# Atten4Vis/LW-DETR

Measured on AMD Instinct MI355X. Metric: images/sec, higher is better.
Workload: dtype fp16; 1 GPU; LW-DETR-small inference forward + PostProcess, 640x640, batch 32/GPU, fp16, random-init weights (synthetic COCO-shaped input); global_batch=32, per_gpu_batch=32, parallelism=dp1, collective=none, launch_chains=2

## Files before the change

### include/lwdetr_hip.h

```cpp
#ifndef LWDETR_HIP_H
#define LWDETR_HIP_H
#include <stdint.h>
#ifdef __cplusplus
extern "C" {
#endif

#define LWDETR_OK 0
#define LWDETR_ERR_BAD_ARG (-1)
#define LWDETR_ERR_UNSUPPORTED (-2)
#define LWDETR_ERR_LAUNCH (-3)

int lwdetr_msda_forward(const void* value, const int64_t* shapes, const int64_t* level_start, const void* loc,
                        const void* attn, void* out, int B, int S, int M, int D, int L, int Q, int P, int dtype,
                        void* hip_stream);

int lwdetr_msda_backward(const void* value, const int64_t* shapes, const int64_t* level_start, const void* loc,
                         const void* attn, const void* grad_out, void* grad_value, void* grad_loc, void* grad_attn,
                         int B, int S, int M, int D, int L, int Q, int P, int dtype, void* hip_stream);

int lwdetr_msda_fused_forward(const void* value, const int64_t* shapes, const int64_t* level_start, const void* oa,
                              long ld_oa, int logit_col, const float* ref_boxes, const float* valid_ratios, void* out,
                              int B, int S, int M, int D, int L, int Q, int P, int dtype, void* hip_stream);

typedef struct {
// ... 27 lines not shown
    const float* ln_stats;
    const float* ln_colsum;
} lwdetr_gemm_seg;

typedef struct {
    const void* A; const void* A2;
    const void* W;
    int M, N, K;
    long lda;
    int a_mode;
    lwdetr_tok_layout a_tok;
    int conv_cin, conv_stride, a_col0, conv_hout, conv_wout;
    int img_h, img_w;
    int nseg;
    lwdetr_gemm_seg seg[3];
    void* splitk_ws;
    int splitk;
} lwdetr_gemm_desc;

int lwdetr_gemm(const lwdetr_gemm_desc* desc, int dtype, void* hip_stream);
int lwdetr_gemm_few(const lwdetr_gemm_desc* desc, int dtype, void* hip_stream);
int lwdetr_row_stats(const void* x, long ldx, long M, int C, float eps, float* stats, int dtype, void* hip_stream);
void lwdetr_gemm_tuning(int big_mode);
int lwdetr_has_experiments(void);
void lwdetr_gemm_pt_tuning(int pt_mode);
long lwdetr_gemm_pt_count(void);
int lwdetr_gemm_path_counts(long* out, int n);
const char* lwdetr_gemm_path_name(int i);

typedef struct {
    const void* Q;
    const void* K;
    const void* VT;
    void* out;
    long ldo;
    int B, heads, hd, Tp;
    int seqs_per_img;
    int seq_tok_stride;
    int keys_per_seq;
    int sub_stride, sub_len;
    int kind;
    int vt_slack;
} lwdetr_attn_desc;

int lwdetr_attention(const lwdetr_attn_desc* desc, int dtype, void* hip_stream);
void lwdetr_attention_tuning(int lds_mode);
// ... 122 lines not shown
typedef struct { int kind; int n; int flags; float eps; void* out; long ldo; } lwdetr_chain_stage;
typedef struct {
    const void* in; long ld_in; int k_in;
    const void* res; long ld_res;
    const void* qpos; long ld_q;
    const void* wstream; const float* vec;
    long M; int D; int nst;
    lwdetr_chain_stage st[6];
} lwdetr_chain_desc;
long lwdetr_row_chain_pieces(const lwdetr_chain_desc* desc);
long lwdetr_row_chain_vec_floats(const lwdetr_chain_desc* desc);
int lwdetr_row_chain(const lwdetr_chain_desc* desc, int dtype, void* hip_stream);

long lwdetr_vit_qkv_stream_bytes(int C);
long lwdetr_vit_qkv_vec_floats(int C);
int lwdetr_vit_qkv(const void* x, long ldx, const void* wstream, const float* vec, long M, int C, float eps, void* q_out,
                   void* k_out, void* vt_out, float qscale, int heads, int hd, int Tp, int dtype, void* hip_stream);

long lwdetr_vit_stem_stream_bytes(int C);
long lwdetr_vit_stem_vec_floats(int C);
int lwdetr_vit_stem(const void* img, int B, int img_h, int img_w, int Hp, int Wp, int Twp, const void* pos, long ldpos, void* x,
                    long ldx, const void* wstream, const float* vec, long M, int C, float eps, void* q_out, void* k_out,
                    void* vt_out, float qscale, int heads, int hd, int dtype, void* hip_stream);

int lwdetr_select_gather(const void* om, const void* enc_cls, long ldc, const float* props, const int64_t* idx,
                         void* om_sel, void* logits_out, float* props_sel, int B, int S, int d, int nq, int ncls,
                         int dtype, void* hip_stream);
int lwdetr_decoder_inputs(const void* enc_delta, const float* props_sel, const float* refpoint, const float* valid_ratios,
                          int L, const void* query_feat, const float* dim_t, void* enc_boxes_out, float* ref_out,
                          void* sine_out, void* xdec_out, int B, int nq, int d, int dtype, void* hip_stream);
int lwdetr_box_reparam(const void* delta, const float* ref, long ref_rows, void* out, long R, int dtype, void* hip_stream);
int lwdetr_finalize_outputs(const void* delta, const float* ref, long ref_rows, void* coord_out, long R, const void* logits_pad,
                            long ldc, int ncls, void* logits_out, long out_layer_rows, int dtype, void* hip_stream);

int lwdetr_rowmax(const void* x, long ld, long rows, int ncols, float* out, int dtype, void* hip_stream);
int lwdetr_topk(const void* x, int B, int N, int K, int64_t* idx_out, float* val_out, int dtype, void* hip_stream);
int lwdetr_postprocess(const void* logits, const void* boxes, const float* target_sizes, int B, int nq, int ncls, int K,
                       float* scores, int64_t* labels, float* out_boxes, int dtype, void* hip_stream);
int lwdetr_postprocess_packed(const void* logits, const void* boxes, const float* target_sizes, int B, int nq, int ncls, int K,
                              float* packed, int dtype, void* hip_stream);

#define LWDETR_CRIT_MAX_LAYERS 8
#define LWDETR_MATCH_MAX_NQ 1024
#define LWDETR_CRIT_QCHUNK 32
typedef struct {
    const void* logits;
// ... 145 lines not shown
```

### lw-detr_amd/_native.py

```python
import ctypes as C
import os

import torch

_HERE = os.path.dirname(os.path.abspath(__file__))
LIB_PATH = os.environ.get("LWDETR_HIP_LIB") or os.path.join(_HERE, "liblwdetr_hip.so")
_lib = None

DT_F32, DT_F16, DT_BF16, DT_F64 = 0, 1, 2, 3
A_PLAIN, A_CONV3x3, A_PATCH16 = 0, 1, 2
ACT_NONE, ACT_RELU, ACT_GELU, ACT_SILU = 0, 1, 2, 3
OUT_LINEAR, OUT_HEADS, OUT_HEADS_T, OUT_TOKMAP, OUT_DECONV2x2 = 0, 1, 2, 3, 4
ERR_BAD_ARG, ERR_UNSUPPORTED, ERR_LAUNCH = -1, -2, -3
ERRORS = {-1: "bad argument", -2: "unsupported configuration", -3: "kernel launch failed"}


class NativeError(RuntimeError):
    pass


class TokLayout(C.Structure):
    _fields_ = [("winmajor", C.c_int), ("Hp", C.c_int), ("Wp", C.c_int), ("Twp", C.c_int)]


# ... 135 lines not shown
        l.lwdetr_attention_tuning_cfg.argtypes = [i]
        l.lwdetr_attention_tuning_cfg.restype = None
        l.lwdetr_layernorm.argtypes = [vp, lg, vp, vp, vp, lg, lg, i, f, lg, lg, lg, i, vp]
        l.lwdetr_layernorm_chain.argtypes = [vp, lg, vp, vp, f, vp, lg, vp, vp, f, vp, lg, lg, i, i, vp]
        l.lwdetr_row_stats.argtypes = [vp, lg, lg, i, f, vp, i, vp]
        l.lwdetr_ffn_splits.argtypes = [lg, i, i, i]
        l.lwdetr_ffn_partial.argtypes = [vp, lg, vp, vp, vp, vp, lg, i, i, i, vp]
        l.lwdetr_ffn_finish.argtypes = [vp, lg, vp, i, vp, vp, vp, f, vp, lg, vp, vp, f, vp, lg, lg, i, i, vp]
        l.lwdetr_mlp_fused.argtypes = [vp, lg, vp, vp, vp, vp, vp, vp, lg, vp, lg, i, f, f, vp, lg, vp, vp, vp,
                                       vp, vp, vp, vp, vp, f, i, i, i, i, vp]
        l.lwdetr_vit_block_few.argtypes = [vp, lg, vp, vp, vp, vp, vp, vp, lg, vp, lg, i, f, f, vp, lg, vp, vp, vp,
                                       vp, vp, vp, vp, vp, f, i, i, i, i, vp]
        l.lwdetr_vit_block.argtypes = [vp, lg, vp, lg, vp, vp, vp, lg, vp, lg, i, f, f, i, vp, vp, vp, f, i, i, i, i, vp]
        l.lwdetr_vit_block_stream_bytes.argtypes = [i, i]
        l.lwdetr_vit_block_stream_bytes.restype = C.c_long
        l.lwdetr_vit_block_vec_floats.argtypes = [i]
        l.lwdetr_vit_block_vec_floats.restype = C.c_long
        l.lwdetr_vit_qkv.argtypes = [vp, lg, vp, vp, lg, i, f, vp, vp, vp, f, i, i, i, i, vp]
        l.lwdetr_vit_stem.argtypes = [vp, i, i, i, i, i, i, vp, lg, vp, lg, vp, vp, lg, i, f, vp, vp, vp, f, i, i, i, vp]
        l.lwdetr_vit_stem_stream_bytes.argtypes = [i]
        l.lwdetr_vit_stem_stream_bytes.restype = C.c_long
        l.lwdetr_vit_stem_vec_floats.argtypes = [i]
        l.lwdetr_vit_stem_vec_floats.restype = C.c_long
        l.lwdetr_vit_qkv_stream_bytes.argtypes = [i]
        l.lwdetr_vit_qkv_stream_bytes.restype = C.c_long
        l.lwdetr_vit_qkv_vec_floats.argtypes = [i]
        l.lwdetr_vit_qkv_vec_floats.restype = C.c_long
        l.lwdetr_enc_chain.argtypes = [vp, lg, i, vp, vp, vp, lg, vp, vp, i, vp, vp, vp, vp, lg, i, i, i, i, lg, i, f, f, i, vp]
        l.lwdetr_enc_chain_vec_floats.argtypes = [i, i]
        l.lwdetr_enc_chain_vec_floats.restype = C.c_long
        l.lwdetr_enc_chain_pieces.argtypes = [i, i, i]
        l.lwdetr_enc_chain_pieces.restype = C.c_long
        l.lwdetr_enc_chain_class_cols.argtypes = [i]
        l.lwdetr_enc_chain_class_cols.restype = C.c_long
        l.lwdetr_enc_chain_vec_floats_cls.argtypes = [i, i, i]
        l.lwdetr_enc_chain_vec_floats_cls.restype = C.c_long
        l.lwdetr_enc_chain_pieces_cls.argtypes = [i, i, i, i]
        l.lwdetr_enc_chain_pieces_cls.restype = C.c_long
        l.lwdetr_enc_chain_check.argtypes = [vp, lg, i, vp, vp, vp, lg, vp, vp, i, vp, vp, vp, vp, lg, i, i, i, i, lg, i, i]
        l.lwdetr_row_chain.argtypes = [C.POINTER(ChainDesc), i, vp]
        l.lwdetr_row_chain_pieces.argtypes = [C.POINTER(ChainDesc)]
        l.lwdetr_row_chain_pieces.restype = C.c_long
        l.lwdetr_row_chain_vec_floats.argtypes = [C.POINTER(ChainDesc)]
        l.lwdetr_row_chain_vec_floats.restype = C.c_long
        l.lwdetr_select_gather.argtypes = [vp, vp, lg, vp, vp, vp, vp, vp, i, i, i, i, i, i, vp]
        l.lwdetr_decoder_inputs.argtypes = [vp, vp, vp, vp, i, vp, vp, vp, vp, vp, vp, i, i, i, i, vp]
# ... 210 lines not shown
```

### lw-detr_amd/csrc/common.h

```cpp
#pragma once
#include <hip/hip_runtime.h>
#include <stdint.h>
#include "lwdetr_hip.h"

enum { DT_F32 = 0, DT_F16 = 1, DT_BF16 = 2 };

typedef _Float16 f16;
typedef __bf16 bf16;
typedef float f32x4 __attribute__((ext_vector_type(4)));
typedef float f32x8 __attribute__((ext_vector_type(8)));
typedef float f32x16 __attribute__((ext_vector_type(16)));
typedef _Float16 f16x4 __attribute__((ext_vector_type(4)));
typedef _Float16 f16x8 __attribute__((ext_vector_type(8)));
typedef __bf16 bf16x4 __attribute__((ext_vector_type(4)));
typedef __bf16 bf16x8 __attribute__((ext_vector_type(8)));
typedef short s16x4 __attribute__((ext_vector_type(4)));

template <typename T> struct Vec;
template <> struct Vec<float> { typedef f32x4 v4; typedef f32x8 v8; };
template <> struct Vec<f16> { typedef f16x4 v4; typedef f16x8 v8; };
template <> struct Vec<bf16> { typedef bf16x4 v4; typedef bf16x8 v8; };

template <typename T> __device__ __forceinline__ float to_f32(T x) { return (float)x; }
template <typename T> __device__ __forceinline__ T from_f32(float x) { return (T)x; }
// ... 92 lines not shown
}
__device__ __forceinline__ long tok_encode(int b, int y, int x, const TokLayout& L) {
    if (!L.winmajor) return ((long)b * L.Hp + y) * L.Wp + x;
    const int h = L.Hp >> 2, w = L.Wp >> 2;
    const int wy = y / h, wx = x / w;
    return (long)b * 16 * L.Twp + (wy * 4 + wx) * L.Twp + (y - wy * h) * w + (x - wx * w);
}

enum {
    KID_MSDA = 0, KID_MSDA_GENERIC, KID_MSDA_FUSED, KID_GEMM, KID_GEMM_CONV, KID_GEMM_PATCH, KID_ATTN_WINDOW,
    KID_ATTN_GLOBAL, KID_ATTN_DECODER, KID_LAYERNORM, KID_ELTWISE, KID_MLP, KID_VITBLOCK, KID_CHAIN, KID_COUNT
};
void lwdetr_prof_begin(int kid, double flops, double bytes, hipStream_t s);
void lwdetr_prof_end(hipStream_t s);
struct ProfScope {
    hipStream_t s;
    ProfScope(int kid, double flops, double bytes, hipStream_t st) : s(st) { lwdetr_prof_begin(kid, flops, bytes, st); }
    ~ProfScope() { lwdetr_prof_end(s); }
};

enum {
    KNOB_ATTN_LDS_CFG = 0, KNOB_ATTN_LDS, KNOB_ATTN_SHORT, KNOB_ATTN_WTILE, KNOB_ATTN_WIN, KNOB_ATTN_QT, KNOB_CHAIN_SPLIT_ROWS, KNOB_GEMM_BIG,
    KNOB_GEMM_BIG_BN, KNOB_GEMM_BIG_2WG, KNOB_CONV_PATCH, KNOB_GEMM_TILE, KNOB_GEMM_DMA, KNOB_GEMM_KB, KNOB_GEMM_NST, KNOB_GEMM_PT,
    KNOB_GEMM_PT_SKEW, KNOB_MLP_SMALL_TT, KNOB_FFN_SPLITS, KNOB_MLP_SMALL, KNOB_VB_GRID, KNOB_VB_GELU16, KNOB_VB_HALF, KNOB_GEMM_FEW_WAVES, KNOB_COUNT
};
long lwdetr_knob(int id, long dflt);
bool lwdetr_knob_is_set(int id);

static inline int lwdetr_check_launch() {
    hipError_t e = hipGetLastError();
    return e == hipSuccess ? LWDETR_OK : LWDETR_ERR_LAUNCH;
}

enum {
    GP_PLAIN_64x64 = 0, GP_PLAIN_128x64, GP_PLAIN_128x128,
    GP_RING_64x64_D2, GP_RING_64x64_D3, GP_RING_64x64_D4, GP_RING_64x64_D3_KB64, GP_RING_64x64_SPLITK, GP_RING_128x64, GP_RING_128x128_D3,
    GP_RING_128x128_D4, GP_CONV_PATCH_128, GP_CONV_PATCH_192,
    GP_BIG_256_KB64, GP_BIG_256_KB32, GP_BIG_192_KB64, GP_BIG_128_KB64, GP_BIG_128_KB32, GP_BIG4_256, GP_BIG4_192, GP_BIG_LN,
    GP_PT, GP_FEW_PLAIN, GP_FEW_CONV_KCH4, GP_FEW_CONV_KCH6, GP_COUNT
};
int lwdetr_gemm_path_done(int path, int rc);
```

### lw-detr_amd/csrc/gemm.hip

```cpp
#include "common.h"
#include <cstdlib>
#include <atomic>
#include <type_traits>

int lwdetr_gemm_pt_try(const lwdetr_gemm_desc& d, int dtype, hipStream_t st, bool& taken);

namespace {

constexpr int BK = 32;

template <typename T> __device__ __forceinline__ float act_apply(float x, int act) {
    if (act == ACT_GELU) return gelu_for<T>(x);
    if (act == ACT_SILU) return x * __builtin_amdgcn_rcpf(1.f + __expf(-x));
    if (act == ACT_RELU) return x > 0.f ? x : 0.f;
    return x;
}

__device__ __forceinline__ bool row_offset(const lwdetr_gemm_seg& sg, long m, long& off) {
    if (sg.mode == LWDETR_OUT_LINEAR) { off = m * sg.ldo; return true; }
    if (sg.mode == LWDETR_OUT_HEADS) {
        const int b = (int)(m / sg.p0), t = (int)(m - (long)b * sg.p0);
        off = ((long)b * sg.p2 * sg.p0 + t) * sg.p1;
        return true;
    }
// ... 1344 lines not shown
    if (state[dev] < 0) { (void)hipGetLastError(); return LWDETR_ERR_UNSUPPORTED; }
    static_assert(NW == 8 || lds <= 80 * 1024, "two workgroups per CU");
    const long nwg = ((d.M + BM - 1) / BM) * ((d.N + BN - 1) / BN);
#ifdef LWDETR_EXPERIMENTS
    if constexpr (LN) hipLaunchKernelGGL((gemm_big_ln_kernel<T>), dim3((unsigned)nwg), dim3(512), lds, st, d);
    else if constexpr (NW == 4) hipLaunchKernelGGL((gemm_big4_kernel<T, BN, KB, NST, AMODE>), dim3((unsigned)nwg), dim3(256), lds, st, d);
    else
#endif
    hipLaunchKernelGGL((gemm_big_kernel<T, BN, KB, NST, AMODE>), dim3((unsigned)nwg), dim3(512), lds, st, d);
    constexpr int path = LN ? GP_BIG_LN
                       : NW == 4 ? (BN == 256 ? GP_BIG4_256 : GP_BIG4_192)
                       : BN == 256 ? (KB == 64 ? GP_BIG_256_KB64 : GP_BIG_256_KB32)
                       : BN == 192 ? GP_BIG_192_KB64 : (KB == 64 ? GP_BIG_128_KB64 : GP_BIG_128_KB32);
    static_assert(NW == 4 || BN != 192 || KB == 64, "one 192-wide 8-wave form");
    return lwdetr_gemm_path_done(path, lwdetr_check_launch());
}

int g_big_mode = -1;
template <int AMODE>
bool big_2wg_pays(const lwdetr_gemm_desc& d, int bn) {
    (void)d; (void)bn;
    return false;
}
template <typename T, int AMODE>
int try_launch_big(const lwdetr_gemm_desc& d, hipStream_t st, bool& taken) {
    taken = false;
    if constexpr (sizeof(T) != 2 || AMODE == LWDETR_A_PATCH16) return LWDETR_OK;
    else {
        const int mode = g_big_mode >= 0 ? g_big_mode : (int)lwdetr_knob(KNOB_GEMM_BIG, 1);
        if (!mode || d.A2 || d.K % 64 != 0 || d.N < 128) return LWDETR_OK;
        if (AMODE == LWDETR_A_CONV3x3 && (d.conv_cin % 64 != 0 || d.a_col0 % 8 != 0 || d.conv_hout > 1024 || d.conv_wout > 1024 ||
                                          d.M / ((long)d.conv_hout * d.conv_wout) >= 2048)) return LWDETR_OK;
        int bn = d.N % 256 == 0 || d.N > 512 ? 256 : (d.N <= 192 ? 192 : 128);
        bn = (int)lwdetr_knob(KNOB_GEMM_BIG_BN, bn);
        for (int s = 0; s < d.nseg; ++s)
            if (d.seg[s].n_begin % bn != 0) bn = 128;
        for (int s = 0; s < d.nseg; ++s) if (d.seg[s].n_begin % bn != 0) return LWDETR_OK;
        const long tiles = ((d.M + 255) / 256) * ((d.N + bn - 1) / bn);
        if (mode == 1 && !(d.K >= 384 && d.N >= 192 && (d.M >= 16384 || (d.K >= 960 && tiles >= 96)))) return LWDETR_OK;
        const int variant = mode >= 10 ? mode : 0;
        const int wg2_mode = (int)lwdetr_knob(KNOB_GEMM_BIG_2WG, 1);
        const bool wg2 = variant == 128 || (variant == 0 && (wg2_mode == 2 || (wg2_mode == 1 && big_2wg_pays<AMODE>(d, bn))));
        int rc;
        bool ln = false;
        for (int s_ = 0; s_ < d.nseg; ++s_) ln = ln || d.seg[s_].ln_stats != nullptr;
        if (ln) {
#ifdef LWDETR_EXPERIMENTS
            if constexpr (AMODE == LWDETR_A_PLAIN) {
                if (bn == 256) { rc = launch_big<T, 256, 64, 2, LWDETR_A_PLAIN, 256, 8, true>(d, st); taken = rc != LWDETR_ERR_UNSUPPORTED; return taken ? rc : LWDETR_OK; }
            }
#endif
            return LWDETR_OK;
        }
#ifdef LWDETR_EXPERIMENTS
        if (wg2 && bn == 256) rc = launch_big<T, 256, 32, 3, AMODE, 128, 4>(d, st);
        else if (wg2 && bn == 192) rc = launch_big<T, 192, 32, 3, AMODE, 128, 4>(d, st);
        else
#else
        (void)wg2;
#endif
        if (bn == 256) rc = variant == 32 ? launch_big<T, 256, 32, 4, AMODE>(d, st) : launch_big<T, 256, 64, 2, AMODE>(d, st);
        else if (bn == 192) rc = launch_big<T, 192, 64, 2, AMODE>(d, st);
        else rc = variant == 32 ? launch_big<T, 128, 32, 4, AMODE>(d, st) : launch_big<T, 128, 64, 3, AMODE>(d, st);
        taken = rc != LWDETR_ERR_UNSUPPORTED;
        return taken ? rc : LWDETR_OK;
    }
}

// ... 125 lines not shown
}

namespace {
std::atomic<long> g_gemm_path[GP_COUNT];
const char* const kGemmPathNames[GP_COUNT] = {
    "gemm_kernel_64x64", "gemm_kernel_128x64", "gemm_kernel_128x128",
    "gemm_dma_64x64_d2", "gemm_dma_64x64_d3", "gemm_dma_64x64_d4", "gemm_dma_64x64_d3_kb64", "gemm_dma_64x64_splitk", "gemm_dma_128x64",
    "gemm_dma_128x128_d3", "gemm_dma_128x128_d4", "conv3x3_patch_128", "conv3x3_patch_192",
    "gemm_big_256_kb64", "gemm_big_256_kb32", "gemm_big_192_kb64", "gemm_big_128_kb64", "gemm_big_128_kb32", "gemm_big4_256", "gemm_big4_192",
    "gemm_big_ln", "gemm_pt", "gemm_few_plain", "gemm_few_conv_kch4", "gemm_few_conv_kch6"};
}

int lwdetr_gemm_path_done(int path, int rc) {
    if (rc == LWDETR_OK && path >= 0 && path < GP_COUNT) g_gemm_path[path].fetch_add(1, std::memory_order_relaxed);
    return rc;
}
extern "C" int lwdetr_gemm_path_counts(long* out, int n) {
    for (int i = 0; out && i < n && i < GP_COUNT; ++i) out[i] = g_gemm_path[i].load(std::memory_order_relaxed);
    return GP_COUNT;
}
extern "C" const char* lwdetr_gemm_path_name(int i) { return i >= 0 && i < GP_COUNT ? kGemmPathNames[i] : nullptr; }

extern "C" void lwdetr_gemm_tuning(int big_mode) { g_big_mode = big_mode; }
extern "C" int lwdetr_has_experiments(void) {
#ifdef LWDETR_EXPERIMENTS
    return 1;
#else
    return 0;
#endif
}

extern "C" int lwdetr_gemm(const lwdetr_gemm_desc* desc, int dtype, void* hip_stream) {
    if (!desc) return LWDETR_ERR_BAD_ARG;
    const lwdetr_gemm_desc& d = *desc;
    if (d.M < 0 || d.N <= 0 || d.K <= 0 || d.K % BK != 0 || !d.A || !d.W) return LWDETR_ERR_BAD_ARG;
    if (d.M == 0) return LWDETR_OK;
    if (d.nseg < 1 || d.nseg > 3 || d.seg[0].n_begin != 0) return LWDETR_ERR_BAD_ARG;
    const int esz = dtype == DT_F32 ? 4 : 2;
    const int epc = 16 / esz;
    for (int s = 0; s < d.nseg; ++s) {
        const lwdetr_gemm_seg& g = d.seg[s];
        if (!g.out || g.n_end <= g.n_begin) return LWDETR_ERR_BAD_ARG;
        if (g.act < LWDETR_ACT_NONE || g.act > LWDETR_ACT_SILU) return LWDETR_ERR_BAD_ARG;
        if (s + 1 < d.nseg && d.seg[s + 1].n_begin != g.n_end) return LWDETR_ERR_BAD_ARG;
        if ((g.mode == LWDETR_OUT_HEADS || g.mode == LWDETR_OUT_HEADS_T) &&
            (g.p0 <= 0 || g.p1 <= 0 || g.p2 <= 0 || g.p1 % 4 != 0 || g.p0 % 4 != 0)) return LWDETR_ERR_BAD_ARG;
// ... 22 lines not shown
```

### lw-detr_amd/csrc/prof.hip

```cpp
#include "common.h"
#include <cstdio>
#include <cstdlib>
#include <cstring>
#include <mutex>
#include <vector>

namespace {
struct Rec { hipEvent_t a, b; int kid; double flops, bytes; };
std::mutex g_mu;
std::vector<Rec> g_open;
std::vector<Rec> g_done;
bool g_on = false;
const char* kNames[KID_COUNT] = {
    "msda_forward_vec8", "msda_forward_generic", "msda_fused_forward", "gemm_mfma", "gemm_mfma_conv3x3",
    "gemm_mfma_patch", "attn_window", "attn_global", "attn_decoder", "layernorm_rows", "eltwise", "mlp_fused", "vit_block", "row_chain"};
}

void lwdetr_prof_begin(int kid, double flops, double bytes, hipStream_t s) {
    if (!g_on) return;
    Rec r; r.kid = kid; r.flops = flops; r.bytes = bytes;
    if (hipEventCreate(&r.a) != hipSuccess || hipEventCreate(&r.b) != hipSuccess) return;
    (void)hipEventRecord(r.a, s);
    std::lock_guard<std::mutex> lk(g_mu);
    g_open.push_back(r);
// ... 21 lines not shown

const char* lwdetr_prof_kernel_name(int kid) { return (kid >= 0 && kid < KID_COUNT) ? kNames[kid] : ""; }

int lwdetr_prof_collect(double* ms, double* flops, double* bytes, long long* count, int n) {
    std::lock_guard<std::mutex> lk(g_mu);
    if (n < KID_COUNT) return LWDETR_ERR_BAD_ARG;
    for (Rec& r : g_done) {
        float t = 0.f;
        if (hipEventSynchronize(r.b) == hipSuccess && hipEventElapsedTime(&t, r.a, r.b) == hipSuccess) {
            ms[r.kid] += t; flops[r.kid] += r.flops; bytes[r.kid] += r.bytes; count[r.kid] += 1;
        }
        (void)hipEventDestroy(r.a); (void)hipEventDestroy(r.b);
    }
    g_done.clear();
    return LWDETR_OK;
}

}

namespace {
const char* kKnobNames[KNOB_COUNT] = {
    "ATTN_LDS_CFG", "ATTN_LDS", "ATTN_SHORT", "ATTN_WTILE", "ATTN_WIN", "ATTN_QT", "CHAIN_SPLIT_ROWS", "GEMM_BIG", "GEMM_BIG_BN", "GEMM_BIG_2WG",
    "CONV_PATCH", "GEMM_TILE", "GEMM_DMA", "GEMM_KB", "GEMM_NST", "GEMM_PT", "GEMM_PT_SKEW", "MLP_SMALL_TT", "FFN_SPLITS", "MLP_SMALL", "VB_GRID",
    "VB_GELU16", "VB_HALF", "GEMM_FEW_WAVES"};
struct KnobTable {
    long val[KNOB_COUNT]; bool set[KNOB_COUNT];
    KnobTable() {
        for (int i = 0; i < KNOB_COUNT; ++i) {
            char name[64];
            snprintf(name, sizeof(name), "LWDETR_%s", kKnobNames[i]);
            const char* e = getenv(name);
            set[i] = e != nullptr && *e != 0;
            val[i] = !set[i] ? 0 : (i == KNOB_VB_GRID && !strcmp(e, "rounds") ? -1 : atol(e));
        }
    }
};
KnobTable& knobs() { static KnobTable t; return t; }
}

long lwdetr_knob(int id, long dflt) { const KnobTable& t = knobs(); return id >= 0 && id < KNOB_COUNT && t.set[id] ? t.val[id] : dflt; }
bool lwdetr_knob_is_set(int id) { return id >= 0 && id < KNOB_COUNT && knobs().set[id]; }

extern "C" int lwdetr_tuning_set(const char* name, long value, int is_set) {
    if (!name) return LWDETR_ERR_BAD_ARG;
    if (!strncmp(name, "LWDETR_", 7)) name += 7;
    for (int i = 0; i < KNOB_COUNT; ++i)
        if (!strcmp(name, kKnobNames[i])) { KnobTable& t = knobs(); t.val[i] = value; t.set[i] = is_set != 0; return LWDETR_OK; }
// ... 3 lines not shown
```

### lw-detr_amd/csrc/vitblock.hip

```cpp
#include "common.h"
#include <atomic>
#include <cstdlib>
#include <cstring>
#include <type_traits>

#ifndef LWDETR_VB_ABLATE
#define LWDETR_VB_ABLATE 0
#endif
#ifdef LWDETR_VB_TIMING
__device__ unsigned long long g_vb_timing[2][4][16];
#define VB_TS(i) do { if ((blockIdx.x == 0 || blockIdx.x == gridDim.x - 1) && lane == 0) { g_vb_timing[blockIdx.x != 0][wave][i] = __builtin_amdgcn_s_memrealtime(); \
    if ((i) == 0) g_vb_timing[blockIdx.x != 0][wave][12] = __builtin_amdgcn_s_memtime(); if ((i) == 11) g_vb_timing[blockIdx.x != 0][wave][15] = __builtin_amdgcn_s_memtime(); } } while (0)
extern "C" int lwdetr_debug_vb_timing(unsigned long long* out) {
    return hipMemcpyFromSymbol(out, HIP_SYMBOL(g_vb_timing), sizeof(g_vb_timing)) == hipSuccess ? 0 : 1;
}
#else
#define VB_TS(i) do {} while (0)
#endif

namespace {

template <typename T> struct Mma32;
template <> struct Mma32<f16> {
    static __device__ __forceinline__ f32x16 k16(f16x8 a, f16x8 b, f32x16 c) { return __builtin_amdgcn_mfma_f32_32x32x16_f16(a, b, c, 0, 0, 0); }
// ... 893 lines not shown
    int dev = 0;
    if (hipGetDevice(&dev) != hipSuccess || dev < 0 || dev >= 16) return LWDETR_ERR_LAUNCH;
    if (!attr_done[dev]) {
        if (hipFuncSetAttribute((const void*)vit_qkv_kernel<T, C, NH>, hipFuncAttributeMaxDynamicSharedMemorySize, (int)lds) != hipSuccess)
            return LWDETR_ERR_LAUNCH;
        attr_done[dev] = true;
    }
    const long per_wg = 4L * 32 * NH;
    long grid = (p.M + per_wg - 1) / per_wg;
    while (((p.M / 8 + grid * 4 - 1) / (grid * 4)) * 8 > 32 * NH) ++grid;
    ProfScope ps(KID_VITBLOCK, 6.0 * p.M * C * C, (double)p.M * C * sizeof(T) * 4, st);
    hipLaunchKernelGGL((vit_qkv_kernel<T, C, NH>), dim3((unsigned)grid), dim3(256), lds, st, p);
    return vit_path_done(vq_path<T, C>(18), lwdetr_check_launch());
}


struct VsParams {
    const void* img; unsigned img_bytes; int img_h, img_w;
    int Hp, Wp, Twp;
    const void* pos; long ldpos;
    VbParams v;
};

template <typename T, int C, int NH>
__global__ __launch_bounds__(256, 1) void vit_stem_kernel(const VsParams ps) {
    typedef typename Vec<T>::v8 V8;
    static_assert(sizeof(T) == 2, "16-bit types only");
    const VbParams& p = ps.v;
    constexpr int KS = C / 16, NTI = C / 32;
    constexpr int PIECE_B = KS * 1024, DPW = KS / 4;
    constexpr int NSLOT = C == 192 ? 8 : 5;
    constexpr int VEC_B = (4 * C * 4 + 4095) / 4096 * 4096, VEC_DPW = VEC_B / 4096;
    constexpr int NP_PE = 24, NP_QKV = 3 * NTI, NP = NP_PE + NP_QKV, Q0 = NP_PE;
    constexpr int NSTEP = NP_PE / 2;
    constexpr int NPX = NH * 4;
    constexpr int PF = 2;
    constexpr int RD = NH == 2 ? 4 : 8;
    static_assert(DPW % 3 == 0 && KS == 2 * NTI, "wait counts are kept in multiples of 3");
    extern __shared__ __attribute__((aligned(16))) char smem[];
    const float* vec = (const float*)(smem + NSLOT * PIECE_B);
    const float* bpe = vec; const float* bqs = vec + C;
    const int tid = threadIdx.x, lane = tid & 63, wave = __builtin_amdgcn_readfirstlane(tid >> 6);
    const int j = lane & 31, h = lane >> 5;
    const unsigned lane16 = lane * 16;
    const unsigned lds0 = (unsigned)(uintptr_t)(__attribute__((address_space(3))) const void*)smem;
    const long U = p.M >> 3, nwv = (long)gridDim.x * 4, wg = (long)blockIdx.x * 4 + wave;
    const long u0 = wg * U / nwv, u1 = (wg + 1) * U / nwv;
    const long t0 = u0 * 8;
    const int nvalid = (int)(u1 - u0) * 8;
    const char* wsrc = (const char*)p.wstream;
    auto dma1k = [&](const char* src_uniform, unsigned voff, unsigned lds_dst) {
        const unsigned lo = __builtin_amdgcn_readfirstlane((unsigned)(uintptr_t)src_uniform);
        const unsigned hi = __builtin_amdgcn_readfirstlane((unsigned)((uintptr_t)src_uniform >> 32));
        const char* sp = (const char*)(((uintptr_t)hi << 32) | lo);
        const unsigned m0v = __builtin_amdgcn_readfirstlane(lds_dst);
        asm volatile("s_mov_b32 m0, %0\n\ts_nop 0\n\tglobal_load_lds_dwordx4 %1, %2" :: "s"(m0v), "v"(voff), "s"(sp) : "memory");
    };
    auto dma_piece = [&](int piece) {
        const unsigned slot = (unsigned)piece % NSLOT;
        const char* src = wsrc + (size_t)piece * PIECE_B;
#pragma unroll
        for (int i = 0; i < DPW; ++i) {
            const unsigned kb = (unsigned)(wave * DPW + i) * 1024u;
            dma1k(src, kb + lane16, lds0 + slot * PIECE_B + kb);
        }
    };
    int issued = 0;
    auto boundary = [&](int a, int b, int extra) {
        __builtin_amdgcn_sched_barrier(0);
        vb_wait_le<12>((issued - b) * DPW + extra);
        asm volatile("s_waitcnt lgkmcnt(0)" ::: "memory");
        __builtin_amdgcn_s_barrier();
        int lim = a + NSLOT; lim = lim < NP ? lim : NP;
        while (issued < lim) { dma_piece(issued); ++issued; }
    };
    auto frag = [&](int piece, int f) -> V8 { return *(const V8*)(smem + ((unsigned)piece % NSLOT) * PIECE_B + f * 1024 + lane16); };
    {
        const char* vsrc = (const char*)p.vec;
#pragma unroll
        for (int i = 0; i < VEC_DPW; ++i) {
            const unsigned kb = (unsigned)(wave * VEC_DPW + i) * 1024u;
            dma1k(vsrc, kb + lane16, lds0 + NSLOT * PIECE_B + kb);
        }
        for (; issued < NSLOT; ++issued) dma_piece(issued);
    }
    const __amdgpu_buffer_rsrc_t r_img = __builtin_amdgcn_make_buffer_rsrc((void*)ps.img, 0, (int)ps.img_bytes, 0x00020000);
    const __amdgpu_buffer_rsrc_t r_pos = __builtin_amdgcn_make_buffer_rsrc((void*)ps.pos, 0, (int)(p.Tp * ps.ldpos * 2), 0x00020000);
    T* x_w = (T*)p.x + t0 * p.ldx;
    const __amdgpu_buffer_rsrc_t r_x = __builtin_amdgcn_make_buffer_rsrc((void*)x_w, 0, (int)(nvalid * p.ldx * 2), 0x00020000);
    unsigned pix0[NH], prow[NH];
    {
        TokLayout L; L.winmajor = 1; L.Hp = ps.Hp; L.Wp = ps.Wp; L.Twp = ps.Twp;
#pragma unroll
// ... 43 lines not shown
#pragma unroll
                    for (int bb = 0; bb < 2; ++bb) {
                        const int b = 2 * jb + bb, c0 = 32 * n + 8 * b + 4 * h;
                        const f32x4 bbv = *(const f32x4*)(bpe + c0);
#pragma unroll
                        for (int d = 0; d < 2; ++d) {
                            const unsigned ow_ = own[2 * bb + d];
                            const typename Pk<T>::v2 v2 = __builtin_bit_cast(typename Pk<T>::v2, ow_);
                            na[th][4 * b + 2 * d] = to_f32<T>(v2[0]) + bbv[2 * d];
                            na[th][4 * b + 2 * d + 1] = to_f32<T>(v2[1]) + bbv[2 * d + 1];
                        }
                    }
                }
#pragma unroll
            for (int th = 0; th < NH; ++th) {
                asm volatile("" : "+a"(na[th]));
                acc2[n][th] = na[th];
            }
            __builtin_amdgcn_sched_barrier(0);
        }
    }
    vb_static_for<NSTEP>([&](auto s_tag) {
        constexpr int s = decltype(s_tag)::value;
        if constexpr (s > 0) {
            constexpr int npos = s < 4 ? NH * NTI * 2 : 0;
            constexpr int hi = s + 1 < NSTEP - 1 ? s + 1 : NSTEP - 1;
            constexpr int lo = s < 4 ? 0 : s - 1;
            boundary(2 * s, 2 * s + 2, npos + (hi - lo + 1) * NPX);
        }
        if constexpr (s + PF < NSTEP) load_px(std::integral_constant<int, s + PF>{});
        V8 fr[RD];
#pragma unroll
        for (int i = 0; i < RD; ++i) fr[i] = frag(2 * s + i / KS, i % KS);
#pragma unroll
        for (int fi = 0; fi < 2 * KS; ++fi) {
            const int kk = fi / NTI, n = fi % NTI;
            const V8 a = fr[fi % RD];
#pragma unroll
            for (int th = 0; th < NH; ++th) acc2[n][th] = Mma32<T>::k16(a, px[s % (PF + 1)][th][kk], acc2[n][th]);
            if (fi + RD < 2 * KS) fr[fi % RD] = frag(2 * s + (fi + RD) / KS, (fi + RD) % KS);
            __builtin_amdgcn_sched_barrier(0);
        }
    });
    V8 xf[NH][KS];
#pragma unroll
    for (int th = 0; th < NH; ++th) {
        float sm = 0.f;
// ... 126 lines not shown
                for (int t = 0; t < KS; ++t) {
                    const V8 a = fr[t % RD];
#pragma unroll
                    for (int th = 0; th < NH; ++th) acc[th] = Mma32<T>::k16(xf[th][t], a, t == 0 ? binit : acc[th]);
                    if (t + RD < KS) fr[t % RD] = frag(piece, t + RD);
                    __builtin_amdgcn_sched_barrier(0);
                }
                const int f = nl0 + j, hh = f >> p.hd_log2, dd = f & (hd - 1);
                const unsigned rowb = (unsigned)(((long)hh * hd + dd) * p.Tp);
#pragma unroll
                for (int th = 0; th < NH; ++th)
#pragma unroll
                    for (int jb = 0; jb < 2; ++jb) {
                        const u32x4 ow = vb_rows8(pack2<T>(acc[th][8 * jb], acc[th][8 * jb + 1]), pack2<T>(acc[th][8 * jb + 2], acc[th][8 * jb + 3]),
                                                  pack2<T>(acc[th][8 * jb + 4], acc[th][8 * jb + 5]), pack2<T>(acc[th][8 * jb + 6], acc[th][8 * jb + 7]));
                        const unsigned off = row_v8[th][jb] == 0x7fffffffu ? 0x80000000u : (row_v8[th][jb] + rowb) * 2u;
                        __builtin_amdgcn_raw_buffer_store_b128(ow, r_v, off, 0, 0);
                    }
            }
        }
    }
}

template <typename T, int C, int NH>
int launch_vs(const VsParams& p, hipStream_t st) {
    constexpr int KS = C / 16, PIECE_B = KS * 1024, NSLOT = C == 192 ? 8 : 5;
    constexpr int VEC_B = (4 * C * 4 + 4095) / 4096 * 4096;
    constexpr size_t lds = (size_t)NSLOT * PIECE_B + VEC_B;
    static bool attr_done[16] = {};
    int dev = 0;
    if (hipGetDevice(&dev) != hipSuccess || dev < 0 || dev >= 16) return LWDETR_ERR_LAUNCH;
    if (!attr_done[dev]) {
        if (hipFuncSetAttribute((const void*)vit_stem_kernel<T, C, NH>, hipFuncAttributeMaxDynamicSharedMemorySize, (int)lds) != hipSuccess)
            return LWDETR_ERR_LAUNCH;
        attr_done[dev] = true;
    }
    const long M = p.v.M, per_wg = 4L * 32 * NH;
    long grid = (M + per_wg - 1) / per_wg;
    while (((M / 8 + grid * 4 - 1) / (grid * 4)) * 8 > 32 * NH) ++grid;
    ProfScope ps(KID_VITBLOCK, (2.0 * 768 + 6.0 * C) * M * C, (double)M * 768 * sizeof(T) + (double)M * C * sizeof(T) * 5, st);
    hipLaunchKernelGGL((vit_stem_kernel<T, C, NH>), dim3((unsigned)grid), dim3(256), lds, st, p);
    return vit_path_done(vq_path<T, C>(22), lwdetr_check_launch());
}

struct VbLaunchState { bool attr_done; int ncu; };

template <typename T, int C, int NH, bool QKV, int WPC = 1, bool G16 = false>
int launch_vb(const VbParams& p, hipStream_t st) {
    constexpr int KS = C / 16, PIECE_B = KS * 1024, NSLOT = WPC == 2 ? 5 : (C == 192 ? 8 : 5);
    constexpr int VEC_B = (13 * C * 4 + 4095) / 4096 * 4096;
    constexpr size_t lds = (size_t)NSLOT * PIECE_B + VEC_B;
    static VbLaunchState state[16] = {};
    int dev = 0;
    if (hipGetDevice(&dev) != hipSuccess || dev < 0 || dev >= 16) return LWDETR_ERR_LAUNCH;
    VbLaunchState& s = state[dev];
    if (!s.attr_done) {
        if (hipFuncSetAttribute((const void*)vitblock_kernel<T, C, NH, QKV, WPC, G16>, hipFuncAttributeMaxDynamicSharedMemorySize, (int)lds) != hipSuccess)
            return LWDETR_ERR_LAUNCH;
        hipDeviceProp_t prop;
        if (hipGetDeviceProperties(&prop, dev) != hipSuccess) return LWDETR_ERR_LAUNCH;
        s.ncu = prop.multiProcessorCount > 0 ? prop.multiProcessorCount : 256;
        s.attr_done = true;
    }
    const long per_wg = 4L * 32 * NH;
    const long need = (p.M + per_wg - 1) / per_wg;
    const long gknob = lwdetr_knob(KNOB_VB_GRID, 0);
    long grid = need;
    if (gknob == -1) grid = (need + s.ncu - 1) / s.ncu * s.ncu;
    else if (gknob >= need) grid = gknob;
    while (((p.M / 8 + grid * 4 - 1) / (grid * 4)) * 8 > 32 * NH) ++grid;
    ProfScope ps(KID_VITBLOCK, (16.0 + 2.0 + (QKV ? 6.0 : 0.0)) * p.M * C * C,
                 (double)p.M * C * sizeof(T) * 3 + (QKV ? 3.0 : 0.0) * p.M * C * sizeof(T) + (p.out2 ? 1.0 : 0.0) * p.M * C * sizeof(T), st);
    hipLaunchKernelGGL((vitblock_kernel<T, C, NH, QKV, WPC, G16>), dim3((unsigned)grid), dim3(256), lds, st, p);
    return vit_path_done(vb_path<T, C, NH, QKV, WPC, G16>(), lwdetr_check_launch());
}

template <typename T>
int dispatch_vb(const VbParams& p, int C, bool qkv, hipStream_t st) {
    const bool g16 = std::is_same<T, f16>::value && lwdetr_knob(KNOB_VB_GELU16, 1) == 1;
    if (C == 192) {
        int dev = 0; (void)hipGetDevice(&dev);
        static int ncu[16] = {};
        if (dev >= 0 && dev < 16 && ncu[dev] == 0) { hipDeviceProp_t prop; ncu[dev] = hipGetDeviceProperties(&prop, dev) == hipSuccess && prop.multiProcessorCount > 0 ? prop.multiProcessorCount : 256; }
        const long cus = dev >= 0 && dev < 16 ? ncu[dev] : 256;
        const bool half = lwdetr_knob_is_set(KNOB_VB_HALF) ? lwdetr_knob(KNOB_VB_HALF, 0) == 1 : (p.M + 127) / 128 <= 2 * cus;
        if (half) {
            if constexpr (sizeof(T) == 2 && std::is_same<T, f16>::value)
                if (g16) return qkv ? launch_vb<T, 192, 1, true, 2, true>(p, st) : launch_vb<T, 192, 1, false, 2, true>(p, st);
            return qkv ? launch_vb<T, 192, 1, true, 2>(p, st) : launch_vb<T, 192, 1, false, 2>(p, st);
        }
    }
    if constexpr (std::is_same<T, f16>::value) {
        if (g16 && C == 192) return qkv ? launch_vb<T, 192, 2, true, 1, true>(p, st) : launch_vb<T, 192, 2, false, 1, true>(p, st);
        if (g16 && C == 384) return qkv ? launch_vb<T, 384, 1, true, 1, true>(p, st) : launch_vb<T, 384, 1, false, 1, true>(p, st);
    }
    if (C == 192) return qkv ? launch_vb<T, 192, 2, true>(p, st) : launch_vb<T, 192, 2, false>(p, st);
    if (C == 384) return qkv ? launch_vb<T, 384, 1, true>(p, st) : launch_vb<T, 384, 1, false>(p, st);
    return LWDETR_ERR_UNSUPPORTED;
}

}

extern "C" int lwdetr_vit_path_counts(long* out, int n) {
    for (int i = 0; out && i < n && i < VP_COUNT; ++i) out[i] = g_vit_path[i].load(std::memory_order_relaxed);
    return VP_COUNT;
}
extern "C" const char* lwdetr_vit_path_name(int i) { return i >= 0 && i < VP_COUNT ? kVitPathNames[i] : nullptr; }
// ... 46 lines not shown
extern "C" long lwdetr_vit_qkv_stream_bytes(int C) { return (C == 192 || C == 384) ? 3L * (C / 32) * (C / 16) * 1024L : -LWDETR_ERR_UNSUPPORTED; }
extern "C" long lwdetr_vit_qkv_vec_floats(int C) { return ((3L * C * 4 + 4095) / 4096 * 4096) / 4; }

extern "C" int lwdetr_vit_qkv(const void* x, long ldx, const void* wstream, const float* vec, long M, int C, float eps, void* q_out,
                              void* k_out, void* vt_out, float qscale, int heads, int hd, int Tp, int dtype, void* hip_stream) {
    if (!x || !wstream || !vec || !q_out || !k_out || !vt_out || M < 0) return LWDETR_ERR_BAD_ARG;
    if (M == 0) return LWDETR_OK;
    if (ldx % 8 != 0 || ((uintptr_t)x | (uintptr_t)wstream | (uintptr_t)vec | (uintptr_t)q_out | (uintptr_t)k_out | (uintptr_t)vt_out) % 16 != 0) return LWDETR_ERR_BAD_ARG;
    if (heads <= 0 || hd < 8 || (hd & (hd - 1)) != 0 || heads * hd != C || Tp <= 0 || Tp % 8 != 0) return LWDETR_ERR_UNSUPPORTED;
    if (M % 8 != 0 || M % Tp != 0 || (double)M * C * 2.0 >= 2147483000.0 || (double)ldx * 64 * 2 >= 2147483000.0) return LWDETR_ERR_UNSUPPORTED;
    if (ldx < C || vb_qkv_overlap(q_out, k_out, vt_out, M, C)) return LWDETR_ERR_BAD_ARG;
    VbParams p = {};
    p.x = (void*)x; p.ldx = ldx; p.wstream = wstream; p.vec = vec; p.M = M; p.eps_next = eps; p.qscale = qscale;
    int l2 = 0; while ((1 << l2) < hd) ++l2;
    p.q = q_out; p.k = k_out; p.vt = vt_out; p.heads = heads; p.hd_log2 = l2; p.Tp = Tp;
    p.qkv_bytes = (unsigned)((unsigned long)M * C * 2ul);
    hipStream_t st = (hipStream_t)hip_stream;
    if (C == 192) return dtype == DT_F16 ? launch_vq<f16, 192, 2>(p, st) : dtype == DT_BF16 ? launch_vq<bf16, 192, 2>(p, st) : LWDETR_ERR_UNSUPPORTED;
    if (C == 384) return dtype == DT_F16 ? launch_vq<f16, 384, 1>(p, st) : dtype == DT_BF16 ? launch_vq<bf16, 384, 1>(p, st) : LWDETR_ERR_UNSUPPORTED;
    return LWDETR_ERR_UNSUPPORTED;
}

extern "C" long lwdetr_vit_stem_stream_bytes(int C) { return (C == 192 || C == 384) ? (24L + 3L * (C / 32)) * (C / 16) * 1024L : -LWDETR_ERR_UNSUPPORTED; }
extern "C" long lwdetr_vit_stem_vec_floats(int C) { return ((4L * C * 4 + 4095) / 4096 * 4096) / 4; }

extern "C" int lwdetr_vit_stem(const void* img, int B, int img_h, int img_w, int Hp, int Wp, int Twp, const void* pos, long ldpos, void* x,
                               long ldx, const void* wstream, const float* vec, long M, int C, float eps, void* q_out, void* k_out,
                               void* vt_out, float qscale, int heads, int hd, int dtype, void* hip_stream) {
    if (!img || !pos || !x || !wstream || !vec || !q_out || !k_out || !vt_out || M < 0 || B <= 0) return LWDETR_ERR_BAD_ARG;
    if (M == 0) return LWDETR_OK;
    const int Tp = 16 * Twp;
    if (img_h != 16 * Hp || img_w != 16 * Wp || Hp % 4 != 0 || Wp % 4 != 0 || Twp < (Hp / 4) * (Wp / 4) || M != (long)B * Tp) return LWDETR_ERR_BAD_ARG;
    if (ldx % 8 != 0 || ldpos % 8 != 0 ||
        ((uintptr_t)img | (uintptr_t)pos | (uintptr_t)x | (uintptr_t)wstream | (uintptr_t)vec | (uintptr_t)q_out | (uintptr_t)k_out | (uintptr_t)vt_out) % 16 != 0)
        return LWDETR_ERR_BAD_ARG;
    if (heads <= 0 || hd < 8 || (hd & (hd - 1)) != 0 || heads * hd != C || Tp % 8 != 0) return LWDETR_ERR_UNSUPPORTED;
    if ((double)M * C * 2.0 >= 2147483000.0 || (double)ldx * 64 * 2 >= 2147483000.0 || (double)B * 3 * img_h * img_w * 2.0 >= 2147483000.0 ||
        (double)Tp * ldpos * 2.0 >= 2147483000.0)
        return LWDETR_ERR_UNSUPPORTED;
    if (ldx < C || ldpos < C || vb_qkv_overlap(q_out, k_out, vt_out, M, C)) return LWDETR_ERR_BAD_ARG;
    VsParams p = {};
    p.img = img; p.img_bytes = (unsigned)((unsigned long)B * 3ul * img_h * img_w * 2ul); p.img_h = img_h; p.img_w = img_w;
    p.Hp = Hp; p.Wp = Wp; p.Twp = Twp; p.pos = pos; p.ldpos = ldpos;
    p.v.x = x; p.v.ldx = ldx; p.v.wstream = wstream; p.v.vec = vec; p.v.M = M; p.v.eps_next = eps; p.v.qscale = qscale;
    int l2 = 0; while ((1 << l2) < hd) ++l2;
    p.v.q = q_out; p.v.k = k_out; p.v.vt = vt_out; p.v.heads = heads; p.v.hd_log2 = l2; p.v.Tp = Tp;
    p.v.qkv_bytes = (unsigned)((unsigned long)M * C * 2ul);
    hipStream_t st = (hipStream_t)hip_stream;
    if (C == 192) return dtype == DT_F16 ? launch_vs<f16, 192, 2>(p, st) : dtype == DT_BF16 ? launch_vs<bf16, 192, 2>(p, st) : LWDETR_ERR_UNSUPPORTED;
    if (C == 384) return dtype == DT_F16 ? launch_vs<f16, 384, 1>(p, st) : dtype == DT_BF16 ? launch_vs<bf16, 384, 1>(p, st) : LWDETR_ERR_UNSUPPORTED;
    return LWDETR_ERR_UNSUPPORTED;
}
```

Before: 14110 images/sec.

## Add two-workgroup-per-CU half-tile ViT stem variant and big-GEMM CU-fill BN rule

Adds a C=192 ViT stem kernel variant that processes half the heads per workgroup (NH=1) with fewer LDS slots, so two workgroups fit per CU. It is selected when the row-tile count is at most twice the CU count, and its wait and prefetch schedule is reworked to match. Separately, the big-GEMM BN choice moves into a helper that drops BN from 256 to 128 when the tile count would fill less than half the CUs, giving more workgroups. The tradeoff is shallower prefetch pipelining in the stem and smaller GEMM tiles with less reuse.

```diff
diff --git a/include/lwdetr_hip.h b/include/lwdetr_hip.h
--- a/include/lwdetr_hip.h
+++ b/include/lwdetr_hip.h
@@ -73,6 +73,7 @@
 int lwdetr_gemm_few(const lwdetr_gemm_desc* desc, int dtype, void* hip_stream);
 int lwdetr_row_stats(const void* x, long ldx, long M, int C, float eps, float* stats, int dtype, void* hip_stream);
 void lwdetr_gemm_tuning(int big_mode);
+int lwdetr_gemm_big_bn(long M, int N, int K, int nseg, const int* seg_begins, int cus, int mode);
 int lwdetr_has_experiments(void);
 void lwdetr_gemm_pt_tuning(int pt_mode);
 long lwdetr_gemm_pt_count(void);
@@ -241,6 +242,7 @@
 int lwdetr_vit_stem(const void* img, int B, int img_h, int img_w, int Hp, int Wp, int Twp, const void* pos, long ldpos, void* x,
                     long ldx, const void* wstream, const float* vec, long M, int C, float eps, void* q_out, void* k_out,
                     void* vt_out, float qscale, int heads, int hd, int dtype, void* hip_stream);
+long lwdetr_vit_stem_half_count(void);
 
 int lwdetr_select_gather(const void* om, const void* enc_cls, long ldc, const float* props, const int64_t* idx,
                          void* om_sel, void* logits_out, float* props_sel, int B, int S, int d, int nq, int ncls,
diff --git a/lw-detr_amd/_native.py b/lw-detr_amd/_native.py
--- a/lw-detr_amd/_native.py
+++ b/lw-detr_amd/_native.py
@@ -181,6 +181,9 @@
         l.lwdetr_vit_stem_stream_bytes.restype = C.c_long
         l.lwdetr_vit_stem_vec_floats.argtypes = [i]
         l.lwdetr_vit_stem_vec_floats.restype = C.c_long
+        l.lwdetr_vit_stem_half_count.argtypes = []
+        l.lwdetr_vit_stem_half_count.restype = C.c_long
+        l.lwdetr_gemm_big_bn.argtypes = [lg, i, i, i, C.POINTER(C.c_int), i, i]
         l.lwdetr_vit_qkv_stream_bytes.argtypes = [i]
         l.lwdetr_vit_qkv_stream_bytes.restype = C.c_long
         l.lwdetr_vit_qkv_vec_floats.argtypes = [i]
diff --git a/lw-detr_amd/csrc/common.h b/lw-detr_amd/csrc/common.h
--- a/lw-detr_amd/csrc/common.h
+++ b/lw-detr_amd/csrc/common.h
@@ -138,7 +138,8 @@
 enum {
     KNOB_ATTN_LDS_CFG = 0, KNOB_ATTN_LDS, KNOB_ATTN_SHORT, KNOB_ATTN_WTILE, KNOB_ATTN_WIN, KNOB_ATTN_QT, KNOB_CHAIN_SPLIT_ROWS, KNOB_GEMM_BIG,
     KNOB_GEMM_BIG_BN, KNOB_GEMM_BIG_2WG, KNOB_CONV_PATCH, KNOB_GEMM_TILE, KNOB_GEMM_DMA, KNOB_GEMM_KB, KNOB_GEMM_NST, KNOB_GEMM_PT,
-    KNOB_GEMM_PT_SKEW, KNOB_MLP_SMALL_TT, KNOB_FFN_SPLITS, KNOB_MLP_SMALL, KNOB_VB_GRID, KNOB_VB_GELU16, KNOB_VB_HALF, KNOB_GEMM_FEW_WAVES, KNOB_COUNT
+    KNOB_GEMM_PT_SKEW, KNOB_MLP_SMALL_TT, KNOB_FFN_SPLITS, KNOB_MLP_SMALL, KNOB_VB_GRID, KNOB_VB_GELU16, KNOB_VB_HALF, KNOB_GEMM_FEW_WAVES,
+    KNOB_VS_HALF, KNOB_GEMM_BIG_FILL, KNOB_COUNT
 };
 long lwdetr_knob(int id, long dflt);
 bool lwdetr_knob_is_set(int id);
diff --git a/lw-detr_amd/csrc/gemm.hip b/lw-detr_amd/csrc/gemm.hip
--- a/lw-detr_amd/csrc/gemm.hip
+++ b/lw-detr_amd/csrc/gemm.hip
@@ -1390,6 +1390,26 @@
     (void)d; (void)bn;
     return false;
 }
+int big_cus() {
+    int dev = 0; (void)hipGetDevice(&dev);
+    static int ncu[16] = {};
+    if (dev >= 0 && dev < 16 && ncu[dev] == 0) { hipDeviceProp_t prop; ncu[dev] = hipGetDeviceProperties(&prop, dev) == hipSuccess && prop.multiProcessorCount > 0 ? prop.multiProcessorCount : 256; }
+    return dev >= 0 && dev < 16 ? ncu[dev] : 256;
+}
+int big_bn_rule(long M, int N, int K, int nseg, const int* seg_begins, int cus, int mode) {
+    if (!mode || K % 64 != 0 || N < 128) return 0;
+    int bn = N % 256 == 0 || N > 512 ? 256 : (N <= 192 ? 192 : 128);
+    bn = (int)lwdetr_knob(KNOB_GEMM_BIG_BN, bn);
+    for (int s = 0; s < nseg; ++s)
+        if (seg_begins[s] % bn != 0) bn = 128;
+    for (int s = 0; s < nseg; ++s) if (seg_begins[s] % bn != 0) return 0;
+    const long tiles = ((M + 255) / 256) * ((N + bn - 1) / bn);
+    if (mode == 1 && !(K >= 384 && N >= 192 && (M >= 16384 || (K >= 960 && tiles >= 96)))) return 0;
+    if (mode == 1 && bn == 256 && N % 128 == 0 && 2 * tiles <= cus && !lwdetr_knob_is_set(KNOB_GEMM_BIG_BN) &&
+        lwdetr_knob(KNOB_GEMM_BIG_2WG, 1) != 2 && lwdetr_knob(KNOB_GEMM_BIG_FILL, 1) != 0)
+        bn = 128;
+    return bn;
+}
 template <typename T, int AMODE>
 int try_launch_big(const lwdetr_gemm_desc& d, hipStream_t st, bool& taken) {
     taken = false;
@@ -1399,19 +1419,15 @@
         if (!mode || d.A2 || d.K % 64 != 0 || d.N < 128) return LWDETR_OK;
         if (AMODE == LWDETR_A_CONV3x3 && (d.conv_cin % 64 != 0 || d.a_col0 % 8 != 0 || d.conv_hout > 1024 || d.conv_wout > 1024 ||
                                           d.M / ((long)d.conv_hout * d.conv_wout) >= 2048)) return LWDETR_OK;
-        int bn = d.N % 256 == 0 || d.N > 512 ? 256 : (d.N <= 192 ? 192 : 128);
-        bn = (int)lwdetr_knob(KNOB_GEMM_BIG_BN, bn);
-        for (int s = 0; s < d.nseg; ++s)
-            if (d.seg[s].n_begin % bn != 0) bn = 128;
-        for (int s = 0; s < d.nseg; ++s) if (d.seg[s].n_begin % bn != 0) return LWDETR_OK;
-        const long tiles = ((d.M + 255) / 256) * ((d.N + bn - 1) / bn);
-        if (mode == 1 && !(d.K >= 384 && d.N >= 192 && (d.M >= 16384 || (d.K >= 960 && tiles >= 96)))) return LWDETR_OK;
+        bool ln = false;
+        int begins[3] = {0, 0, 0};
+        for (int s_ = 0; s_ < d.nseg && s_ < 3; ++s_) { ln = ln || d.seg[s_].ln_stats != nullptr; begins[s_] = d.seg[s_].n_begin; }
+        const int bn = big_bn_rule(d.M, d.N, d.K, d.nseg < 3 ? d.nseg : 3, begins, ln ? 0 : big_cus(), mode);
+        if (!bn) return LWDETR_OK;
         const int variant = mode >= 10 ? mode : 0;
         const int wg2_mode = (int)lwdetr_knob(KNOB_GEMM_BIG_2WG, 1);
         const bool wg2 = variant == 128 || (variant == 0 && (wg2_mode == 2 || (wg2_mode == 1 && big_2wg_pays<AMODE>(d, bn))));
         int rc;
-        bool ln = false;
-        for (int s_ = 0; s_ < d.nseg; ++s_) ln = ln || d.seg[s_].ln_stats != nullptr;
         if (ln) {
 #ifdef LWDETR_EXPERIMENTS
             if constexpr (AMODE == LWDETR_A_PLAIN) {
@@ -1583,6 +1599,10 @@
 extern "C" const char* lwdetr_gemm_path_name(int i) { return i >= 0 && i < GP_COUNT ? kGemmPathNames[i] : nullptr; }
 
 extern "C" void lwdetr_gemm_tuning(int big_mode) { g_big_mode = big_mode; }
+extern "C" int lwdetr_gemm_big_bn(long M, int N, int K, int nseg, const int* seg_begins, int cus, int mode) {
+    if (M < 0 || N <= 0 || K <= 0 || nseg < 0 || nseg > 3 || (nseg > 0 && !seg_begins)) return LWDETR_ERR_BAD_ARG;
+    return big_bn_rule(M, N, K, nseg, seg_begins, cus, mode);
+}
 extern "C" int lwdetr_has_experiments(void) {
 #ifdef LWDETR_EXPERIMENTS
     return 1;
diff --git a/lw-detr_amd/csrc/prof.hip b/lw-detr_amd/csrc/prof.hip
--- a/lw-detr_amd/csrc/prof.hip
+++ b/lw-detr_amd/csrc/prof.hip
@@ -67,7 +67,7 @@
 const char* kKnobNames[KNOB_COUNT] = {
     "ATTN_LDS_CFG", "ATTN_LDS", "ATTN_SHORT", "ATTN_WTILE", "ATTN_WIN", "ATTN_QT", "CHAIN_SPLIT_ROWS", "GEMM_BIG", "GEMM_BIG_BN", "GEMM_BIG_2WG",
     "CONV_PATCH", "GEMM_TILE", "GEMM_DMA", "GEMM_KB", "GEMM_NST", "GEMM_PT", "GEMM_PT_SKEW", "MLP_SMALL_TT", "FFN_SPLITS", "MLP_SMALL", "VB_GRID",
-    "VB_GELU16", "VB_HALF", "GEMM_FEW_WAVES"};
+    "VB_GELU16", "VB_HALF", "GEMM_FEW_WAVES", "VS_HALF", "GEMM_BIG_FILL"};
 struct KnobTable {
     long val[KNOB_COUNT]; bool set[KNOB_COUNT];
     KnobTable() {
diff --git a/lw-detr_amd/csrc/vitblock.hip b/lw-detr_amd/csrc/vitblock.hip
--- a/lw-detr_amd/csrc/vitblock.hip
+++ b/lw-detr_amd/csrc/vitblock.hip
@@ -939,14 +939,15 @@
     VbParams v;
 };
 
-template <typename T, int C, int NH>
-__global__ __launch_bounds__(256, 1) void vit_stem_kernel(const VsParams ps) {
+template <typename T, int C, int NH, int WPC = 1>
+__global__ __launch_bounds__(256, WPC) void vit_stem_kernel(const VsParams ps) {
     typedef typename Vec<T>::v8 V8;
     static_assert(sizeof(T) == 2, "16-bit types only");
+    static_assert(WPC == 1 || (WPC == 2 && C == 192 && NH == 1), "two workgroups per CU: the C = 192 half tile");
     const VbParams& p = ps.v;
     constexpr int KS = C / 16, NTI = C / 32;
     constexpr int PIECE_B = KS * 1024, DPW = KS / 4;
-    constexpr int NSLOT = C == 192 ? 8 : 5;
+    constexpr int NSLOT = WPC == 2 ? 5 : (C == 192 ? 8 : 5);
     constexpr int VEC_B = (4 * C * 4 + 4095) / 4096 * 4096, VEC_DPW = VEC_B / 4096;
     constexpr int NP_PE = 24, NP_QKV = 3 * NTI, NP = NP_PE + NP_QKV, Q0 = NP_PE;
     constexpr int NSTEP = NP_PE / 2;
@@ -985,7 +986,10 @@
     int issued = 0;
     auto boundary = [&](int a, int b, int extra) {
         __builtin_amdgcn_sched_barrier(0);
-        vb_wait_le<12>((issued - b) * DPW + extra);
+        if constexpr (WPC == 2) {
+            const int n = (issued - b) * DPW + extra;
+            vb_wait_le<6>(n - n % 3);
+        } else vb_wait_le<12>((issued - b) * DPW + extra);
         asm volatile("s_waitcnt lgkmcnt(0)" ::: "memory");
         __builtin_amdgcn_s_barrier();
         int lim = a + NSLOT; lim = lim < NP ? lim : NP;
@@ -1075,7 +1079,13 @@
     }
     vb_static_for<NSTEP>([&](auto s_tag) {
         constexpr int s = decltype(s_tag)::value;
-        if constexpr (s > 0) {
+        if constexpr (s > 0 && WPC == 2) {
+            constexpr bool pro = 2 * s + 1 < NSLOT;
+            constexpr int npos = pro ? NH * NTI * 2 : 0;
+            constexpr int hi = s + 1 < NSTEP - 1 ? s + 1 : NSTEP - 1;
+            constexpr int lo = pro ? 0 : (2 * s + 1 - NSLOT) / 2 + 1 + PF;
+            boundary(2 * s, 2 * s + 2, npos + (hi >= lo ? hi - lo + 1 : 0) * NPX);
+        } else if constexpr (s > 0) {
             constexpr int npos = s < 4 ? NH * NTI * 2 : 0;
             constexpr int hi = s + 1 < NSTEP - 1 ? s + 1 : NSTEP - 1;
             constexpr int lo = s < 4 ? 0 : s - 1;
@@ -1248,16 +1258,19 @@
     }
 }
 
-template <typename T, int C, int NH>
+std::atomic<long> g_vs_half;
+
+template <typename T, int C, int NH, int WPC = 1>
 int launch_vs(const VsParams& p, hipStream_t st) {
-    constexpr int KS = C / 16, PIECE_B = KS * 1024, NSLOT = C == 192 ? 8 : 5;
+    constexpr int KS = C / 16, PIECE_B = KS * 1024, NSLOT = WPC == 2 ? 5 : (C == 192 ? 8 : 5);
     constexpr int VEC_B = (4 * C * 4 + 4095) / 4096 * 4096;
     constexpr size_t lds = (size_t)NSLOT * PIECE_B + VEC_B;
+    static_assert(WPC == 1 || lds <= 80 * 1024, "two workgroups per CU");
     static bool attr_done[16] = {};
     int dev = 0;
     if (hipGetDevice(&dev) != hipSuccess || dev < 0 || dev >= 16) return LWDETR_ERR_LAUNCH;
     if (!attr_done[dev]) {
-        if (hipFuncSetAttribute((const void*)vit_stem_kernel<T, C, NH>, hipFuncAttributeMaxDynamicSharedMemorySize, (int)lds) != hipSuccess)
+        if (hipFuncSetAttribute((const void*)vit_stem_kernel<T, C, NH, WPC>, hipFuncAttributeMaxDynamicSharedMemorySize, (int)lds) != hipSuccess)
             return LWDETR_ERR_LAUNCH;
         attr_done[dev] = true;
     }
@@ -1265,8 +1278,10 @@
     long grid = (M + per_wg - 1) / per_wg;
     while (((M / 8 + grid * 4 - 1) / (grid * 4)) * 8 > 32 * NH) ++grid;
     ProfScope ps(KID_VITBLOCK, (2.0 * 768 + 6.0 * C) * M * C, (double)M * 768 * sizeof(T) + (double)M * C * sizeof(T) * 5, st);
-    hipLaunchKernelGGL((vit_stem_kernel<T, C, NH>), dim3((unsigned)grid), dim3(256), lds, st, p);
-    return vit_path_done(vq_path<T, C>(22), lwdetr_check_launch());
+    hipLaunchKernelGGL((vit_stem_kernel<T, C, NH, WPC>), dim3((unsigned)grid), dim3(256), lds, st, p);
+    const int rc = vit_path_done(vq_path<T, C>(22), lwdetr_check_launch());
+    if (WPC == 2 && rc == LWDETR_OK) g_vs_half.fetch_add(1, std::memory_order_relaxed);
+    return rc;
 }
 
 struct VbLaunchState { bool attr_done; int ncu; };
@@ -1301,14 +1316,18 @@
     return vit_path_done(vb_path<T, C, NH, QKV, WPC, G16>(), lwdetr_check_launch());
 }
 
+long vit_cus() {
+    int dev = 0; (void)hipGetDevice(&dev);
+    static int ncu[16] = {};
+    if (dev >= 0 && dev < 16 && ncu[dev] == 0) { hipDeviceProp_t prop; ncu[dev] = hipGetDeviceProperties(&prop, dev) == hipSuccess && prop.multiProcessorCount > 0 ? prop.multiProcessorCount : 256; }
+    return dev >= 0 && dev < 16 ? ncu[dev] : 256;
+}
+
 template <typename T>
 int dispatch_vb(const VbParams& p, int C, bool qkv, hipStream_t st) {
     const bool g16 = std::is_same<T, f16>::value && lwdetr_knob(KNOB_VB_GELU16, 1) == 1;
     if (C == 192) {
-        int dev = 0; (void)hipGetDevice(&dev);
-        static int ncu[16] = {};
-        if (dev >= 0 && dev < 16 && ncu[dev] == 0) { hipDeviceProp_t prop; ncu[dev] = hipGetDeviceProperties(&prop, dev) == hipSuccess && prop.multiProcessorCount > 0 ? prop.multiProcessorCount : 256; }
-        const long cus = dev >= 0 && dev < 16 ? ncu[dev] : 256;
+        const long cus = vit_cus();
         const bool half = lwdetr_knob_is_set(KNOB_VB_HALF) ? lwdetr_knob(KNOB_VB_HALF, 0) == 1 : (p.M + 127) / 128 <= 2 * cus;
         if (half) {
             if constexpr (sizeof(T) == 2 && std::is_same<T, f16>::value)
@@ -1401,6 +1420,7 @@
 }
 
 extern "C" long lwdetr_vit_stem_stream_bytes(int C) { return (C == 192 || C == 384) ? (24L + 3L * (C / 32)) * (C / 16) * 1024L : -LWDETR_ERR_UNSUPPORTED; }
+extern "C" long lwdetr_vit_stem_half_count(void) { return g_vs_half.load(std::memory_order_relaxed); }
 extern "C" long lwdetr_vit_stem_vec_floats(int C) { return ((4L * C * 4 + 4095) / 4096 * 4096) / 4; }
 
 extern "C" int lwdetr_vit_stem(const void* img, int B, int img_h, int img_w, int Hp, int Wp, int Twp, const void* pos, long ldpos, void* x,
@@ -1426,7 +1446,12 @@
     p.v.q = q_out; p.v.k = k_out; p.v.vt = vt_out; p.v.heads = heads; p.v.hd_log2 = l2; p.v.Tp = Tp;
     p.v.qkv_bytes = (unsigned)((unsigned long)M * C * 2ul);
     hipStream_t st = (hipStream_t)hip_stream;
-    if (C == 192) return dtype == DT_F16 ? launch_vs<f16, 192, 2>(p, st) : dtype == DT_BF16 ? launch_vs<bf16, 192, 2>(p, st) : LWDETR_ERR_UNSUPPORTED;
+    if (C == 192) {
+        const bool half = lwdetr_knob_is_set(KNOB_VS_HALF) ? lwdetr_knob(KNOB_VS_HALF, 0) == 1 : (M + 127) / 128 <= 2 * vit_cus();
+        if (dtype == DT_F16) return half ? launch_vs<f16, 192, 1, 2>(p, st) : launch_vs<f16, 192, 2>(p, st);
+        if (dtype == DT_BF16) return half ? launch_vs<bf16, 192, 1, 2>(p, st) : launch_vs<bf16, 192, 2>(p, st);
+        return LWDETR_ERR_UNSUPPORTED;
+    }
     if (C == 384) return dtype == DT_F16 ? launch_vs<f16, 384, 1>(p, st) : dtype == DT_BF16 ? launch_vs<bf16, 384, 1>(p, st) : LWDETR_ERR_UNSUPPORTED;
     return LWDETR_ERR_UNSUPPORTED;
 }
```

Result: no change. 14050 images/sec (-0.5%).
